# immars/parameter_server

Hardware: AMD Instinct MI355X
Metric: examples/sec (whole node) sparse LR 10^9 feats at 1/2/4/8 MI355X (higher is better)
Workload: dtype fp32; 1 GPU; global_batch=65536, seq_len=39, nnz_per_example=39, parallelism=dp1+kvshard1, consistency=bsp (1 shard: every pull sees every earlier push), table_slots_per_gpu=2147483648, hip_graph=False, collectives_in_graphs=False, prep_streams=3, localize=tpf

## Files before the change

### parameter_server_amd/csrc/hip/tploc.cuh

```cuda
#pragma once
#include "tploc.h"

namespace psamd {

namespace tp {
constexpr int kThr = 1024;
constexpr int kIt = 8;
constexpr int kTile = kThr * kIt;
constexpr int kHash = 2 * kTile;
constexpr int kHB = 14;
constexpr int kDispB = 12;
constexpr uint32_t kMaxDisp = (1u << kDispB) - 1;
constexpr int kMaxBk = 2048;
constexpr int kMaxT = 640;
constexpr int kBThr = 256;
constexpr int kBkThr = 512;
constexpr int kECap = 4096;
constexpr int kECapL = 4064;
constexpr int kDH = 2048;
constexpr int kBkProbe = 128;
constexpr uint32_t kEmpty = 0xffffffffu;
constexpr int kG = (kECapL + kBkThr - 1) / kBkThr;
}

__device__ __forceinline__ uint32_t tp_hash(uint32_t x) {
  x ^= x >> 16;
  x *= 0x7feb352du;
  x ^= x >> 15;
  x *= 0x846ca68bu;
  x ^= x >> 16;
  return x;
}

template <int kN>
__device__ __forceinline__ uint32_t tp_block_scan(uint32_t v, uint32_t* lds, uint32_t* total) {
  constexpr int kW = kN / 64;
  const int lane = threadIdx.x & 63, wid = threadIdx.x >> 6;
  uint32_t x = v;
#pragma unroll
  for (int off = 1; off < 64; off <<= 1) {
    const uint32_t y = __shfl_up(x, off, 64);
    if (lane >= off) x += y;
  }
  if (lane == 63) lds[wid] = x;
  __syncthreads();
  if (threadIdx.x == 0) {
    uint32_t run = 0;
    for (int w = 0; w < kW; ++w) {
      const uint32_t t = lds[w];
      lds[w] = run;
      run += t;
    }
    lds[kW] = run;
  }
  __syncthreads();
  const uint32_t r = x - v + lds[wid];
  *total = lds[kW];
  __syncthreads();
  return r;
}

template <int kN>
__device__ __forceinline__ uint32_t tp_prefix(const uint32_t* __restrict__ a, int b, uint32_t* lds) {
  uint32_t s = 0;
  for (int i = threadIdx.x; i < b; i += kN) s += a[i];
  uint32_t tot;
  tp_block_scan<kN>(s, lds, &tot);
  return tot;
}

__device__ __forceinline__ uint64_t tp_match_any(uint32_t v, int nbits, uint64_t active) {
  uint64_t peers = active;
  for (int b = 0; b < nbits; ++b) {
    const bool bit = (v >> b) & 1u;
    const uint64_t bal = __ballot(bit);
    peers &= bit ? bal : ~bal;
  }
  return peers;
}

template <bool kCnt = false>
__device__ __forceinline__ bool tp_bk_build(const uint32_t* __restrict__ tkeys,
                                            const uint16_t* __restrict__ toff, int nbf, int T,
                                            int shift, int f0, int nf, uint32_t hb,
                                            uint32_t* hkey, uint32_t* hcnt, uint64_t* dl,
                                            uint16_t* eh, uint32_t* lds, uint32_t* flag,
                                            int32_t (&idx)[tp::kG], uint32_t* E_out,
                                            uint32_t* D_out, uint64_t* prof,
                                            const uint8_t* __restrict__ ecnt = nullptr) {
  using namespace tp;
  const int t = threadIdx.x;
  uint32_t* tpre = reinterpret_cast<uint32_t*>(dl);
  uint16_t* tlo = reinterpret_cast<uint16_t*>(tpre + kMaxT + 1);
  uint16_t* tmid = tlo + kMaxT;
  for (int s = t; s < kDH; s += kBkThr) {
    hkey[s] = kEmpty;
    hcnt[s] = 0;
  }
  if (t == 0) *flag = 0;
  const int per = (T + kBkThr - 1) / kBkThr;
  const int q0 = t * per, q1 = q0 + per < T ? q0 + per : T;
  uint32_t c = 0;
  for (int q = q0; q < q1; ++q) {
    const uint16_t* to = toff + (int64_t)q * (nbf + 1);
    const uint32_t lo = to[f0], hi = to[f0 + nf];
    tlo[q] = (uint16_t)lo;
    tmid[q] = (uint16_t)((nf == 2 ? to[f0 + 1] : hi) - lo);
    tpre[q] = hi - lo;
    c += hi - lo;
  }
  uint32_t E;
  uint32_t w = tp_block_scan<kBkThr>(c, lds, &E);
  for (int q = q0; q < q1; ++q) {
    const uint32_t len = tpre[q];
    tpre[q] = w;
    w += len;
  }
  if (t == 0) tpre[T] = E;
  __syncthreads();
  if (prof && t == 0) prof[(int64_t)blockIdx.x * 12 + 1] = clock64();
  const uint32_t En = E < (uint32_t)kECapL ? E : (uint32_t)kECapL;
  bool bad = E > (uint32_t)kECapL;
  uint32_t hib = 0;
#pragma unroll
  for (int q = 0; q < kG; ++q) {
    const uint32_t g = q * kBkThr + t;
    idx[q] = -1;
    if (g < En) {
      int lo = 0, up = T - 1;
      while (lo < up) {
        const int mid = (lo + up + 1) >> 1;
        if (tpre[mid] <= g) lo = mid; else up = mid - 1;
      }
      const uint32_t off = g - tpre[lo];
      idx[q] = lo * kTile + tlo[lo] + (int32_t)off;
      hib |= (off >= tmid[lo] ? 1u : 0u) << q;
    }
  }
  uint32_t kv[kG];
  uint32_t ecp[(kG + 3) / 4];
#pragma unroll
  for (int q = 0; q < kG; ++q) kv[q] = idx[q] >= 0 ? tkeys[idx[q]] : 0u;
  if (kCnt) {
#pragma unroll
    for (int w = 0; w < (kG + 3) / 4; ++w) ecp[w] = 0u;
#pragma unroll
    for (int q = 0; q < kG; ++q)
      if (idx[q] >= 0) ecp[q >> 2] |= (uint32_t)ecnt[idx[q]] << ((q & 3) * 8);
  }
#pragma unroll
  for (int q = 0; q < kG; ++q) {
    if (idx[q] < 0) continue;
    const uint32_t g = q * kBkThr + t;
    const uint32_t key = kv[q] | ((hb + ((hib >> q) & 1u)) << shift);
    uint32_t h = tp_hash(key) & (kDH - 1);
    bool ok = false;
    bad |= __hip_atomic_load(flag, __ATOMIC_RELAXED, __HIP_MEMORY_SCOPE_WORKGROUP) != 0u;
    for (int p = 0; p < kBkProbe && !bad; ++p) {
      const uint32_t cu = hkey[h];
      if (cu == kEmpty) {
        const uint32_t prev = atomicCAS(&hkey[h], kEmpty, key);
        if (prev == kEmpty || prev == key) { ok = true; break; }
      } else if (cu == key) {
        ok = true;
        break;
      }
      h = (h + 1) & (kDH - 1);
    }
    if (ok) {
      atomicAdd(&hcnt[h], kCnt ? (ecp[q >> 2] >> ((q & 3) * 8)) & 0xffu : 1u);
    } else if (!bad) {
      bad = true;
      atomicOr(flag, 1u);
    }
    eh[g] = ok ? (uint16_t)h : (uint16_t)0xffffu;
  }
  if (bad) atomicOr(flag, 1u);
  __syncthreads();
  if (prof && t == 0) prof[(int64_t)blockIdx.x * 12 + 2] = clock64();
  constexpr int kPer = kDH / kBkThr;
  uint64_t ent[kPer];
  uint32_t cc = 0;
#pragma unroll
  for (int q = 0; q < kPer; ++q) {
    const int s = q * kBkThr + t;
    ent[q] = hkey[s] != kEmpty
                 ? (((uint64_t)hkey[s] << 32) |
                    ((uint64_t)(kCnt ? min(hcnt[s], 0xffffu) : hcnt[s]) << 16) | (uint64_t)s)
                 : ~0ull;
    cc += ent[q] != ~0ull;
  }
  uint32_t D;
  uint32_t wd = tp_block_scan<kBkThr>(cc, lds, &D);
#pragma unroll
  for (int q = 0; q < kPer; ++q)
    if (ent[q] != ~0ull) dl[wd++] = ent[q];
  *E_out = En;
  *D_out = D;
  const bool good = *flag == 0u;
  __syncthreads();
  return good;
}

__device__ __forceinline__ void tp_bk_ranksort(uint64_t* dl, uint64_t* hs, uint32_t D) {
  using namespace tp;
  const int t = threadIdx.x;
  if (t < 8 && D + t < (uint32_t)kDH) dl[D + t] = ~0ull;
  uint32_t* rk = reinterpret_cast<uint32_t*>(hs + 1024);
  const int tpk = D <= 128 ? 4 : D <= 256 ? 2 : 1;
  if (tpk > 1 && t < 256) rk[t] = 0;
  __syncthreads();
  const uint4* d4 = reinterpret_cast<const uint4*>(dl);
  const uint32_t nq = (D + 7) / 8;
  if (tpk > 1) {
    const int nk = kBkThr / tpk, i = t % nk, h = t / nk;
    const uint32_t pq = (nq + tpk - 1) / tpk;
    const uint32_t qa = h * pq, qb = qa + pq < nq ? qa + pq : nq;
    if ((uint32_t)i < D) {
      const uint64_t x = dl[i];
      uint32_t r = 0;
      for (uint32_t q = qa; q < qb; ++q) {
        uint4 v[4];
#pragma unroll
        for (int k = 0; k < 4; ++k) v[k] = d4[q * 4 + k];
#pragma unroll
        for (int k = 0; k < 4; ++k) {
          r += (((uint64_t)v[k].y << 32) | v[k].x) < x;
          r += (((uint64_t)v[k].w << 32) | v[k].z) < x;
        }
      }
      atomicAdd(&rk[i], r);
    }
    __syncthreads();
    if (h == 0 && (uint32_t)i < D) hs[rk[i]] = dl[i];
  } else {
    for (uint32_t i = t; i < D; i += kBkThr) {
      const uint64_t x = dl[i];
      uint32_t r = 0;
      for (uint32_t q = 0; q < nq; ++q) {
        uint4 v[4];
#pragma unroll
        for (int k = 0; k < 4; ++k) v[k] = d4[q * 4 + k];
#pragma unroll
        for (int k = 0; k < 4; ++k) {
          r += (((uint64_t)v[k].y << 32) | v[k].x) < x;
          r += (((uint64_t)v[k].w << 32) | v[k].z) < x;
        }
      }
      hs[r] = x;
    }
  }
}

__device__ __forceinline__ int fx_shift(uint32_t maxbits) {
  int e = 0;
  if (maxbits) (void)frexpf(__uint_as_float(maxbits), &e);
  return min(100, 48 - e);
}
__device__ __forceinline__ void fx_add(long long* acc, int idx, float v, double sc) {
  const long long fx = __double2ll_rn((double)v * sc);
  if (fx) atomicAdd(reinterpret_cast<unsigned long long*>(&acc[idx]), (unsigned long long)fx);
}
__device__ __forceinline__ void fx_tile_max(float vmax, uint32_t* smax) {
  vmax = wave_max(vmax);
  if ((threadIdx.x & 63) == 0 && vmax > 0.f) atomicMax(smax, __float_as_uint(vmax));
}

namespace tpf {
constexpr int kUnitK = tp::kDH;
constexpr int kUC = 2 * kUnitK;
constexpr int kEC = 8192;
constexpr int kThr = 256;
constexpr uint32_t kNoSlot = 0xffffffffu;
}

__host__ __device__ __forceinline__ int tpf_xcd_group_of(int bid, int groups) {
  if (groups < 8) return bid;
  const int q = groups >> 3, r = groups & 7, xcd = bid & 7;
  const int base = xcd < r ? xcd * (q + 1) : r * (q + 1) + (xcd - r) * q;
  return base + (bid >> 3);
}

}
```

### parameter_server_amd/csrc/hip/tploc.hip

```cpp
#include "tploc.cuh"
#include "tploc_geom.h"

#include <algorithm>
#include <cstdlib>

namespace psamd {

__device__ uint64_t* g_tile_prof = nullptr;
#define TILE_MARK(k)                                                            \
  if (tpp && threadIdx.x == 0) tpp[(int64_t)blockIdx.x * 16 + (k)] = clock64()

template <bool kQuot, bool kCnt = false>
__global__ void __launch_bounds__(tp::kThr, 8)
tp_tile_kernel(const uint64_t* __restrict__ raw, int64_t n, KeyMix m, int shift, int nbk,
               uint32_t* __restrict__ tkeys, uint16_t* __restrict__ toff,
               int32_t* __restrict__ dcnt, uint16_t* __restrict__ rep,
               int32_t* __restrict__ err, int lts, uint8_t* __restrict__ ecnt = nullptr) {
  using namespace tp;
  __shared__ uint32_t hk[kHash];
  __shared__ uint32_t cnt[kMaxBk];
  __shared__ uint32_t lds[kThr / 64 + 1];
  const int t = threadIdx.x;
  uint64_t* const tpp = g_tile_prof;
  if (tpp && t == 0) tpp[(int64_t)blockIdx.x * 16 + 8] = __builtin_amdgcn_s_memrealtime();
  TILE_MARK(0);
  for (int i = t; i < kHash; i += kThr) hk[i] = kEmpty;
  for (int d = t; d < nbk; d += kThr) cnt[d] = 0;
  __syncthreads();
  TILE_MARK(1);
  const int64_t base = (int64_t)blockIdx.x << lts;
  const int lim = (int)(n - base < (1 << lts) ? n - base : (1 << lts));
  uint64_t kr[kIt];
  uint16_t sl[kIt];
  uint32_t rr[kIt];
  uint32_t won = 0;
  bool bad = false;
#pragma unroll
  for (int j = 0; j < kIt; ++j) {
    const int o = j * kThr + t;
    kr[j] = o < lim ? raw[base + o] : 0ull;
  }
  if (tpp) {
    __builtin_amdgcn_s_waitcnt(0);
    __syncthreads();
    TILE_MARK(2);
  }
#pragma unroll
  for (int j = 0; j < kIt; ++j) {
    sl[j] = 0;
    if (j * kThr + t < lim) {
      const uint64_t k = kQuot ? mix_key(kr[j], m) : (uint64_t)mix_key32(kr[j], m);
      kr[j] = k;
      const uint32_t q = kQuot ? (uint32_t)(k >> kHB) << kDispB : (uint32_t)k;
      uint32_t h = (uint32_t)k & (kHash - 1);
      uint32_t d = 0;
      for (; d < kMaxDisp; ++d) {
        const uint32_t want = kQuot ? q | d : q;
        const uint32_t cur = hk[h];
        if (cur == want) break;
        if (cur == kEmpty) {
          const uint32_t prev = atomicCAS(&hk[h], kEmpty, want);
          if (prev == kEmpty) {
            won |= 1u << j;
            break;
          }
          if (prev == want) break;
        }
        h = (h + 1) & (kHash - 1);
      }
      bad |= d == kMaxDisp;
      sl[j] = (uint16_t)h;
    }
  }
#pragma unroll
  for (int j = 0; j < kIt; ++j)
    rr[j] = (won >> j) & 1u ? atomicAdd(&cnt[kr[j] >> shift], 1u) : kEmpty;
  if (bad && err) atomicOr(err, 2);
  __syncthreads();
  TILE_MARK(3);
  constexpr int kDP = kMaxBk / kThr;
  uint32_t c[kDP], s = 0;
#pragma unroll
  for (int e = 0; e < kDP; ++e) {
    const int d = t * kDP + e;
    c[e] = d < nbk ? cnt[d] : 0u;
    s += c[e];
  }
  uint32_t D;
  uint32_t run = tp_block_scan<kThr>(s, lds, &D);
  uint16_t* to = toff + (int64_t)blockIdx.x * (nbk + 1);
#pragma unroll
  for (int e = 0; e < kDP; ++e) {
    const int d = t * kDP + e;
    if (d < nbk) {
      cnt[d] = run;
      to[d] = (uint16_t)run;
    }
    run += c[e];
  }
  if (t == 0) {
    to[nbk] = (uint16_t)D;
    dcnt[blockIdx.x] = (int32_t)D;
  }
  __syncthreads();
  TILE_MARK(4);
  uint32_t* tk = tkeys + (int64_t)blockIdx.x * kTile;
  const uint64_t smask = (1ull << shift) - 1;
#pragma unroll
  for (int j = 0; j < kIt; ++j) {
    if (rr[j] != kEmpty) {
      const uint32_t pos = cnt[kr[j] >> shift] + rr[j];
      tk[pos] = (uint32_t)(kr[j] & smask);
      hk[sl[j]] = pos;
    }
  }
  __syncthreads();
  TILE_MARK(5);
#pragma unroll
  for (int j = 0; j < kIt; ++j) {
    const int o = j * kThr + t;
    if (o < lim) {
      const uint16_t pos = (uint16_t)hk[sl[j]];
      rep[base + o] = pos;
      if (kCnt) sl[j] = pos;
    }
  }
  if (kCnt) {
    __syncthreads();
    for (uint32_t i = t; i < (D + 1) / 2; i += kThr) hk[i] = 0u;
    __syncthreads();
#pragma unroll
    for (int j = 0; j < kIt; ++j)
      if (j * kThr + t < lim) atomicAdd(&hk[sl[j] >> 1], 1u << ((sl[j] & 1) * 16));
    __syncthreads();
    uint8_t* ec = ecnt + (int64_t)blockIdx.x * kTile;
    for (uint32_t i = t; i < D; i += kThr) {
      const uint32_t c = (hk[i >> 1] >> ((i & 1) * 16)) & 0xffffu;
      ec[i] = (uint8_t)(c > 255u ? 255u : c);
    }
  }
  if (tpp && t == 0) {
    TILE_MARK(6);
    tpp[(int64_t)blockIdx.x * 16 + 9] = __builtin_amdgcn_s_memrealtime();
    tpp[(int64_t)blockIdx.x * 16 + 10] = __smid();
  }
}
#undef TILE_MARK

void tp_tile_set_prof(uint64_t* p) {
  PSAMD_HIP_CHECK(hipMemcpyToSymbol(HIP_SYMBOL(g_tile_prof), &p, sizeof(p)));
}

__global__ void tp_gather_kernel(const uint16_t* __restrict__ rep,
                                 const int32_t* __restrict__ ent_uid, int64_t n,
                                 int32_t* __restrict__ local_col) {
  constexpr int kPer = 4;
  const int64_t i0 = (blockIdx.x * (int64_t)blockDim.x) * kPer + threadIdx.x;
  int64_t e[kPer];
#pragma unroll
  for (int q = 0; q < kPer; ++q) {
    const int64_t i = i0 + q * blockDim.x;
    e[q] = i < n ? (i / tp::kTile) * tp::kTile + rep[i] : -1;
  }
#pragma unroll
  for (int q = 0; q < kPer; ++q) {
    const int64_t i = i0 + q * blockDim.x;
    if (e[q] >= 0) local_col[i] = ent_uid[e[q]];
  }
}

int tp_flat_lts(int64_t n) {
  const char* pe = getenv("PSAMD_TILE_LTS");
  const int pin = pe ? atoi(pe) : 0;
  const char* te = getenv("PSAMD_TILE_MIN");
  int tmin = te ? atoi(te) : 128;
  tmin = tmin < 1 ? 1 : tmin > tp::kMaxT / 2 ? tp::kMaxT / 2 : tmin;
  int lts = 13;
  if (pin >= 10 && pin <= 13) {
    lts = pin;
  } else {
    while (lts > 10 && ((n + (1ll << lts) - 1) >> lts) < tmin) --lts;
  }
  while (lts < 13 && ((n + (1ll << lts) - 1) >> lts) > tp::kMaxT) ++lts;
  return lts;
}

TpGeom tp_geom(int64_t n, int bits, bool flat) {
  TpGeom g;
  g.lts = flat ? tp_flat_lts(n) : 13;
  static_assert(tp::kTile == 8192, "tile entry stride 2^13");
  g.T = (n + (1ll << g.lts) - 1) >> g.lts;
  g.N = g.T * tp::kTile;
  int bb = 0;
  while (bb < 11 && (n >> bb) > 1024) ++bb;
  if (bb > bits) bb = bits;
  g.nbk = 1 << bb;
  g.shift = bits - bb;
  return g;
}

int64_t tploc_stride(int64_t n) { return tp_geom(n, 31).N; }
int64_t tpf_stride(int64_t n) { return tp_geom(n, 31, true).N; }
int64_t tpf_stride_max(int64_t n) {
  const int64_t t = std::min<int64_t>(tp::kMaxT, (n + 1023) / 1024);
  return std::max<int64_t>(t, (n + tp::kTile - 1) / tp::kTile) * tp::kTile;
}
int tpf_tile_log2(int64_t n) { return tp_geom(n, 31, true).lts; }
int tploc_buckets(int64_t n, int bits) { return tp_geom(n, bits).nbk; }
int tploc_tile() { return tp::kTile; }

bool tploc_supported(int64_t n, int bits) {
  return bits >= 2 && bits <= 34 && n > 0 && (n >> 11) <= 1280 &&
         (n + tp::kTile - 1) / tp::kTile <= tp::kMaxT && tp_geom(n, bits).shift <= 31;
}

size_t tploc_temp_bytes(int64_t n, int bits) {
  const TpGeom g = tp_geom(n, bits);
  return al16((size_t)g.nbk * 8 + 16)
         + al16((size_t)g.N * 4)
         + al16((size_t)g.T * (g.nbk + 1) * 2);
}

void tp_launch_tile(const uint64_t* raw, int64_t n, KeyMix m, const TpGeom& g, uint32_t* tkeys,
                    uint16_t* toff, int32_t* dcnt, uint16_t* rep, int32_t* err, uint8_t* ecnt,
                    hipStream_t st) {
  auto launch = [&](auto kernel) {
    kernel<<<(unsigned)g.T, tp::kThr, 0, st>>>(raw, n, m, g.shift, g.nbk, tkeys, toff, dcnt, rep,
                                               err, g.lts, ecnt);
  };
  const bool quot = m.bits > 31;
  if (quot && ecnt) launch(tp_tile_kernel<true, true>);
  else if (ecnt) launch(tp_tile_kernel<false, true>);
  else if (quot) launch(tp_tile_kernel<true, false>);
  else launch(tp_tile_kernel<false, false>);
  PSAMD_HIP_CHECK(hipGetLastError());
}

int tpf_groups(int64_t n, int bits) { return tpf_groups_of(tp_geom(n, bits)); }
int tpf_key_region() { return tpf::kUC; }
int tpf_entry_region() { return tpf::kEC; }
int tpf_xcd_group(int bid, int groups) { return tpf_xcd_group_of(bid, groups); }

size_t tpf_temp_bytes(int64_t n, int bits) {
  const int64_t N = tpf_stride_max(n);
  return al16((size_t)N * 4) + al16((size_t)(N / tp::kTile) * (tp::kMaxBk + 1) * 2);
}

void tp_gather(const uint16_t* rep, const int32_t* ent_uid, int64_t n, int32_t* local_col,
               hipStream_t st) {
  if (n <= 0) return;
  tp_gather_kernel<<<(unsigned)((n + 1023) / 1024), 256, 0, st>>>(rep, ent_uid, n, local_col);
  PSAMD_HIP_CHECK(hipGetLastError());
}

}
```

### parameter_server_amd/csrc/hip/tploc_bucket.hip

```cpp
#include "tploc.cuh"
#include "tploc_geom.h"

#include <stdexcept>

namespace psamd {

namespace tp {
constexpr uint64_t kStA = 1, kStP = 2;
constexpr uint32_t kStM = (1u << 27) - 1;
}
__device__ __forceinline__ uint64_t tp_status(uint32_t ep, uint64_t flag, uint32_t d, uint32_t e) {
  return ((uint64_t)ep << 56) | (flag << 54) | ((uint64_t)(d & tp::kStM) << 27) | (e & tp::kStM);
}

__device__ __forceinline__ void tp_bk_emit(const uint64_t* hs, uint64_t* dl, const uint16_t* eh,
                                           const int32_t (&idx)[tp::kG], uint32_t D,
                                           uint32_t ubase, uint32_t ebase, uint64_t key0,
                                           uint32_t* lds, int32_t* __restrict__ pos_s,
                                           int32_t* __restrict__ segid,
                                           uint64_t* __restrict__ uniq,
                                           int32_t* __restrict__ seg_start,
                                           int32_t* __restrict__ ent_uid,
                                           float* __restrict__ zero_a,
                                           unsigned long long* __restrict__ zero_b,
                                           int64_t u_cap, int64_t e_cap, uint64_t* prof) {
  using namespace tp;
  const int t = threadIdx.x;
  uint32_t* cur = reinterpret_cast<uint32_t*>(dl);
  uint16_t* jj = reinterpret_cast<uint16_t*>(cur + kDH);
  __syncthreads();
  uint32_t carry = 0;
  for (uint32_t j0 = 0; j0 < D; j0 += kBkThr) {
    const uint32_t j = j0 + t;
    const uint64_t v = j < D ? hs[j] : 0ull;
    const uint32_t cnt = (uint32_t)(v >> 16) & 0xffffu;
    uint32_t tot;
    const uint32_t ex = tp_block_scan<kBkThr>(cnt, lds, &tot) + carry;
    if (j < D) {
      const uint32_t slot = (uint32_t)v & 0xffffu;
      const int64_t u = (int64_t)ubase + j;
      if (in_range(u, u_cap)) {
        uniq[u] = key0 | (uint32_t)(v >> 32);
        seg_start[u] = (int32_t)(ebase + ex);
        if (zero_a) zero_a[u] = 0.f;
        if (zero_b) zero_b[u] = 0ull;
      }
      cur[slot] = ex;
      jj[slot] = (uint16_t)j;
    }
    carry += tot;
  }
  __syncthreads();
  if (prof && t == 0) prof[(int64_t)blockIdx.x * 12 + 6] = clock64();
#pragma unroll
  for (int q = 0; q < kG; ++q) {
    if (idx[q] < 0) continue;
    const uint32_t h = eh[q * kBkThr + t];
    if (h == 0xffffu) continue;
    const uint32_t pos = atomicAdd(&cur[h], 1u);
    const uint32_t u = ubase + jj[h];
    const int64_t e = (int64_t)ebase + pos;
    if (in_range(e, e_cap)) {
      pos_s[e] = idx[q];
      segid[e] = (int32_t)(u + 1);
    }
    if (in_range((int64_t)idx[q], e_cap)) ent_uid[idx[q]] = (int32_t)u;
  }
  __syncthreads();
}

__device__ __forceinline__ void tp_bk_lookback(uint64_t* __restrict__ status, int fs, int twin,
                                               int nbf, uint32_t ep, uint32_t D, uint32_t E,
                                               uint32_t* sb, uint32_t* __restrict__ epoch,
                                               int32_t* __restrict__ n_uniq,
                                               int32_t* __restrict__ n_ent,
                                               int32_t* __restrict__ seg_start, int64_t u_cap,
                                               int32_t* __restrict__ err) {
  using namespace tp;
  const int lane = threadIdx.x;
  if (lane >= 64) return;
  uint32_t su = 0, se = 0;
  if (fs > 0) {
    int j = fs - 1;
    uint32_t spins = 0;
    while (true) {
      const int jl = j - lane;
      const uint64_t st =
          jl >= 0 ? __hip_atomic_load(&status[jl], __ATOMIC_RELAXED, __HIP_MEMORY_SCOPE_AGENT)
                  : tp_status(ep, kStP, 0, 0);
      const uint32_t f = (uint32_t)(st >> 56) == ep ? (uint32_t)(st >> 54) & 3u : 0u;
      const uint64_t pm = __ballot(f == kStP), nr = __ballot(f == 0);
      const int fp = pm ? __builtin_ctzll(pm) : 64;
      const uint64_t need = fp >= 63 ? ~0ull : ((2ull << fp) - 1);
      if (nr & need) {
        if (++spins > (1u << 22)) {
          if (lane == 0) atomicOr(err, 4);
          break;
        }
        __builtin_amdgcn_s_sleep(1);
        continue;
      }
      const bool inc = lane <= fp;
      su += wave_allsum(inc ? (uint32_t)(st >> 27) & kStM : 0u);
      se += wave_allsum(inc ? (uint32_t)st & kStM : 0u);
      if (fp < 64) break;
      j -= 64;
    }
  }
  if (lane == 0) {
    const uint64_t inc = tp_status(ep, kStP, su + D, se + E);
    if (fs > 0) __hip_atomic_store(&status[fs], inc, __ATOMIC_RELAXED, __HIP_MEMORY_SCOPE_AGENT);
    if (twin != fs) __hip_atomic_store(&status[twin], inc, __ATOMIC_RELAXED, __HIP_MEMORY_SCOPE_AGENT);
    sb[1] = su;
    sb[2] = se;
    if (twin == nbf - 1) {
      const uint32_t U = su + D, Et = se + E;
      *n_uniq = (int32_t)U;
      *n_ent = (int32_t)Et;
      if (in_range((int64_t)U, u_cap + 1)) seg_start[U] = (int32_t)Et;
      __hip_atomic_store(epoch, ep, __ATOMIC_RELAXED, __HIP_MEMORY_SCOPE_AGENT);
    }
  }
}

__device__ __forceinline__ void tp_bk_fine_light(
    const uint32_t* __restrict__ tkeys, const uint16_t* __restrict__ toff, int nbf, int T,
    int shift, int f, uint32_t hb, uint64_t key0, uint32_t* hkey, uint32_t* hcnt, uint64_t* hs,
    uint64_t* dl, uint16_t* ehraw, uint32_t* lds, uint32_t* sb, uint64_t* __restrict__ status,
    uint32_t ep, uint32_t* __restrict__ epoch, int32_t* __restrict__ pos_s,
    int32_t* __restrict__ segid, uint64_t* __restrict__ uniq, int32_t* __restrict__ seg_start,
    int32_t* __restrict__ ent_uid, int32_t* __restrict__ n_uniq, int32_t* __restrict__ n_ent,
    float* __restrict__ zero_a, unsigned long long* __restrict__ zero_b, int64_t u_cap,
    int64_t e_cap, int32_t* __restrict__ err) {
  using namespace tp;
  static_assert((kMaxT + 1) * 4 + kMaxT * 2 <= kECapL * 2, "tile runs must fit in eh");
  const int t = threadIdx.x;
  uint32_t* tpre = reinterpret_cast<uint32_t*>(ehraw);
  uint16_t* tlo = reinterpret_cast<uint16_t*>(tpre + kMaxT + 1);
  for (int s = t; s < kDH; s += kBkThr) {
    hkey[s] = kEmpty;
    hcnt[s] = 0;
  }
  const int per = (T + kBkThr - 1) / kBkThr;
  const int q0 = t * per, q1 = q0 + per < T ? q0 + per : T;
  uint32_t c = 0;
  for (int q = q0; q < q1; ++q) {
    const uint16_t* to = toff + (int64_t)q * (nbf + 1);
    const uint32_t lo = to[f], hi = to[f + 1];
    tlo[q] = (uint16_t)lo;
    tpre[q] = hi - lo;
    c += hi - lo;
  }
  uint32_t E;
  uint32_t w = tp_block_scan<kBkThr>(c, lds, &E);
  for (int q = q0; q < q1; ++q) {
    const uint32_t len = tpre[q];
    tpre[q] = w;
    w += len;
  }
  if (t == 0) tpre[T] = E;
  __syncthreads();
  auto locate = [&](uint32_t g) -> int32_t {
    int lo = 0, up = T - 1;
    while (lo < up) {
      const int mid = (lo + up + 1) >> 1;
      if (tpre[mid] <= g) lo = mid; else up = mid - 1;
    }
    return lo * kTile + tlo[lo] + (int32_t)(g - tpre[lo]);
  };
  bool bad = false;
  for (uint32_t g = t; g < E; g += kBkThr) {
    const uint32_t key = tkeys[locate(g)] | (hb << shift);
    uint32_t h = tp_hash(key) & (kDH - 1);
    bool ok = false;
    for (int p = 0; p < kBkProbe && !bad; ++p) {
      const uint32_t cu = hkey[h];
      if (cu == kEmpty) {
        const uint32_t prev = atomicCAS(&hkey[h], kEmpty, key);
        if (prev == kEmpty || prev == key) { ok = true; break; }
      } else if (cu == key) {
        ok = true;
        break;
      }
      h = (h + 1) & (kDH - 1);
    }
    if (ok) atomicAdd(&hcnt[h], 1u);
    else bad = true;
  }
  if (bad) atomicOr(err, 1);
  __syncthreads();
  constexpr int kPer = kDH / kBkThr;
  uint32_t cc = 0;
  for (int q = 0; q < kPer; ++q) cc += hkey[q * kBkThr + t] != kEmpty;
  uint32_t D;
  uint32_t wd = tp_block_scan<kBkThr>(cc, lds, &D);
  for (int q = 0; q < kPer; ++q) {
    const int s = q * kBkThr + t;
    if (hkey[s] != kEmpty) dl[wd++] = ((uint64_t)hkey[s] << 32) | ((uint64_t)hcnt[s] << 16) | (uint64_t)s;
  }
  if (t == 0)
    __hip_atomic_store(&status[f], tp_status(ep, f == 0 ? kStP : kStA, D, E), __ATOMIC_RELAXED,
                       __HIP_MEMORY_SCOPE_AGENT);
  __syncthreads();
  tp_bk_ranksort(dl, hs, D);
  tp_bk_lookback(status, f, f, nbf, ep, D, E, sb, epoch, n_uniq, n_ent, seg_start, u_cap, err);
  __syncthreads();
  const uint32_t ubase = sb[1], ebase = sb[2];
  uint32_t* cur = reinterpret_cast<uint32_t*>(dl);
  uint32_t carry = 0;
  for (uint32_t j0 = 0; j0 < D; j0 += kBkThr) {
    const uint32_t j = j0 + t;
    const uint64_t v = j < D ? hs[j] : 0ull;
    const uint32_t cnt = (uint32_t)(v >> 16) & 0xffffu;
    uint32_t tot;
    const uint32_t ex = tp_block_scan<kBkThr>(cnt, lds, &tot) + carry;
    if (j < D) {
      const int64_t u = (int64_t)ubase + j;
      if (in_range(u, u_cap)) {
        uniq[u] = key0 | (uint32_t)(v >> 32);
        seg_start[u] = (int32_t)(ebase + ex);
        if (zero_a) zero_a[u] = 0.f;
        if (zero_b) zero_b[u] = 0ull;
      }
      cur[j] = ex;
    }
    carry += tot;
  }
  __syncthreads();
  for (uint32_t g = t; g < E; g += kBkThr) {
    const int32_t id = locate(g);
    const uint32_t key = tkeys[id] | (hb << shift);
    uint32_t lo = 0, up = D - 1;
    while (lo < up) {
      const uint32_t mid = (lo + up) >> 1;
      if ((uint32_t)(hs[mid] >> 32) < key) lo = mid + 1; else up = mid;
    }
    if (D == 0 || (uint32_t)(hs[lo] >> 32) != key) continue;
    const uint32_t pos = atomicAdd(&cur[lo], 1u);
    const uint32_t u = ubase + lo;
    const int64_t e = (int64_t)ebase + pos;
    if (in_range(e, e_cap)) {
      pos_s[e] = id;
      segid[e] = (int32_t)(u + 1);
    }
    if (in_range((int64_t)id, e_cap)) ent_uid[id] = (int32_t)u;
  }
  __syncthreads();
}

__global__ void __launch_bounds__(tp::kBkThr, 8)
tp_bucket_kernel(const uint32_t* __restrict__ tkeys, const uint16_t* __restrict__ toff, int nbf,
                 int pair, int T, int shift, uint64_t* __restrict__ status,
                 uint32_t* __restrict__ epoch, int32_t* __restrict__ pos_s,
                 int32_t* __restrict__ segid, uint64_t* __restrict__ uniq,
                 int32_t* __restrict__ seg_start, int32_t* __restrict__ ent_uid,
                 int32_t* __restrict__ n_uniq, int32_t* __restrict__ n_ent,
                 float* __restrict__ zero_a, unsigned long long* __restrict__ zero_b,
                 int64_t u_cap, int64_t e_cap, int32_t* __restrict__ err,
                 uint64_t* __restrict__ prof) {
  using namespace tp;
  __shared__ uint16_t eh[kECapL];
  __shared__ uint64_t hs[kDH];
  __shared__ uint64_t dl[kDH];
  __shared__ uint32_t lds[kBkThr / 64 + 1];
  __shared__ uint32_t sb[4];
  static_assert((kMaxT + 1) * 4 + kMaxT * 4 <= kDH * 8, "tile runs must fit in dl");
  uint32_t* hkey = reinterpret_cast<uint32_t*>(hs);
  uint32_t* hcnt = hkey + kDH;
  const int t = threadIdx.x, b = blockIdx.x;
  if (prof && t == 0) {
    prof[(int64_t)b * 12 + 0] = clock64();
    prof[(int64_t)b * 12 + 8] = __builtin_amdgcn_s_memrealtime();
  }
  if (t == 0) {
    uint32_t ep = (__hip_atomic_load(epoch, __ATOMIC_RELAXED, __HIP_MEMORY_SCOPE_AGENT) + 1u) & 0xffu;
    sb[0] = ep ? ep : 1u;
  }
  const int f0 = pair ? 2 * b : b, twin = pair ? f0 + 1 : f0;
  const uint64_t key0 = (uint64_t)f0 << shift;
  int32_t idx[kG];
  uint32_t E, D;
  const bool good = tp_bk_build(tkeys, toff, nbf, T, shift, f0, pair ? 2 : 1, 0u, hkey, hcnt, dl,
                                eh, lds, &sb[3], idx, &E, &D, prof);
  const uint32_t ep = sb[0];
  if (!good && pair) {
#pragma unroll 1
    for (int s = 0; s < 2; ++s)
      tp_bk_fine_light(tkeys, toff, nbf, T, shift, f0 + s, (uint32_t)s, key0, hkey, hcnt, hs, dl,
                       eh, lds, sb, status, ep, epoch, pos_s, segid, uniq, seg_start, ent_uid,
                       n_uniq, n_ent, zero_a, zero_b, u_cap, e_cap, err);
    return;
  }
  if (!good && t == 0) atomicOr(err, 1);
  if (t == 0) {
    if (twin != f0)
      __hip_atomic_store(&status[twin], tp_status(ep, kStA, 0, 0), __ATOMIC_RELAXED,
                         __HIP_MEMORY_SCOPE_AGENT);
    __hip_atomic_store(&status[f0], tp_status(ep, f0 == 0 ? kStP : kStA, D, E), __ATOMIC_RELAXED,
                       __HIP_MEMORY_SCOPE_AGENT);
  }
  if (prof && t == 0) prof[(int64_t)b * 12 + 3] = clock64();
  tp_bk_ranksort(dl, hs, D);
  if (prof && t == 0) prof[(int64_t)b * 12 + 4] = clock64();
  tp_bk_lookback(status, f0, twin, nbf, ep, D, E, sb, epoch, n_uniq, n_ent, seg_start, u_cap, err);
  __syncthreads();
  if (prof && t == 0) prof[(int64_t)b * 12 + 5] = clock64();
  tp_bk_emit(hs, dl, eh, idx, D, sb[1], sb[2], key0, lds, pos_s, segid, uniq, seg_start, ent_uid,
             zero_a, zero_b, u_cap, e_cap, prof);
  if (prof && t == 0) {
    prof[(int64_t)b * 12 + 7] = clock64();
    prof[(int64_t)b * 12 + 9] = __builtin_amdgcn_s_memrealtime();
  }
}

__device__ __forceinline__ uint32_t tpf_unit_light(
    const uint32_t* __restrict__ tkeys, const uint16_t* __restrict__ toff, int nbf, int T,
    int shift, int f, uint32_t hb, uint64_t key0, uint32_t* hkey, uint32_t* hmap,
    uint16_t* ehraw, uint32_t* lds, uint64_t* __restrict__ uo, int32_t* __restrict__ po,
    uint16_t* __restrict__ jo, uint32_t eoff, int32_t* __restrict__ co,
    int32_t* __restrict__ err, bool sorted) {
  using namespace tp;
  const int t = threadIdx.x;
  uint32_t* tpre = reinterpret_cast<uint32_t*>(ehraw);
  uint16_t* tlo = reinterpret_cast<uint16_t*>(tpre + kMaxT + 1);
  for (int s = t; s < kDH; s += kBkThr) hkey[s] = kEmpty;
  const int per = (T + kBkThr - 1) / kBkThr;
  const int q0 = t * per, q1 = q0 + per < T ? q0 + per : T;
  uint32_t c = 0;
  for (int q = q0; q < q1; ++q) {
    const uint16_t* to = toff + (int64_t)q * (nbf + 1);
    const uint32_t lo = to[f], hi = to[f + 1];
    tlo[q] = (uint16_t)lo;
    tpre[q] = hi - lo;
    c += hi - lo;
  }
  uint32_t E;
  uint32_t w = tp_block_scan<kBkThr>(c, lds, &E);
  for (int q = q0; q < q1; ++q) {
    const uint32_t len = tpre[q];
    tpre[q] = w;
    w += len;
  }
  if (t == 0) tpre[T] = E;
  __syncthreads();
  auto locate = [&](uint32_t g) -> int32_t {
    int lo = 0, up = T - 1;
    while (lo < up) {
      const int mid = (lo + up + 1) >> 1;
      if (tpre[mid] <= g) lo = mid; else up = mid - 1;
    }
    return lo * kTile + tlo[lo] + (int32_t)(g - tpre[lo]);
  };
  auto probe = [&](uint32_t key, bool insert) -> int {
    uint32_t h = tp_hash(key) & (kDH - 1);
    for (int p = 0; p < kDH; ++p) {
      const uint32_t cu = hkey[h];
      if (cu == key) return (int)h;
      if (cu == kEmpty) {
        if (!insert) return -1;
        const uint32_t prev = atomicCAS(&hkey[h], kEmpty, key);
        if (prev == kEmpty || prev == key) return (int)h;
      }
      h = (h + 1) & (kDH - 1);
    }
    return -1;
  };
  bool bad = false;
  constexpr int kLB = 4;
  for (uint32_t c0 = 0; c0 < E; c0 += kBkThr * kLB) {
    int32_t id[kLB];
    uint32_t kk[kLB];
#pragma unroll
    for (int q = 0; q < kLB; ++q) {
      const uint32_t g = c0 + q * kBkThr + t;
      id[q] = locate(g < E ? g : E - 1);
    }
#pragma unroll
    for (int q = 0; q < kLB; ++q) kk[q] = tkeys[id[q]];
#pragma unroll
    for (int q = 0; q < kLB; ++q)
      if (c0 + q * kBkThr + t < E) bad |= probe(kk[q] | (hb << shift), true) < 0;
  }
  __syncthreads();
  constexpr int kPer = kDH / kBkThr;
  uint32_t cc = 0;
#pragma unroll
  for (int q = 0; q < kPer; ++q) cc += hkey[q * kBkThr + t] != kEmpty;
  uint32_t D;
  uint32_t wd = tp_block_scan<kBkThr>(cc, lds, &D);
#pragma unroll
  for (int q = 0; q < kPer; ++q) {
    const int s = q * kBkThr + t;
    const uint32_t k = hkey[s];
    if (k != kEmpty) {
      uint32_t j = wd++;
      if (sorted) {
        j = 0;
        for (int r = 0; r < kDH; ++r) j += hkey[r] < k;
      }
      hmap[s] = j;
      uo[j] = key0 | k;
    }
  }
  __syncthreads();
  const uint32_t room = eoff < (uint32_t)tpf::kEC ? tpf::kEC - eoff : 0u;
  bad |= E > room;
  const uint32_t Er = E < room ? E : room;
  for (uint32_t c0 = 0; c0 < Er; c0 += kBkThr * kLB) {
    int32_t id[kLB];
    uint32_t kk[kLB];
#pragma unroll
    for (int q = 0; q < kLB; ++q) {
      const uint32_t g = c0 + q * kBkThr + t;
      id[q] = locate(g < Er ? g : Er - 1);
    }
#pragma unroll
    for (int q = 0; q < kLB; ++q) kk[q] = tkeys[id[q]];
#pragma unroll
    for (int q = 0; q < kLB; ++q) {
      const uint32_t g = c0 + q * kBkThr + t;
      if (g >= Er) continue;
      const int h = probe(kk[q] | (hb << shift), false);
      po[eoff + g] = id[q];
      jo[eoff + g] = h >= 0 ? (uint16_t)hmap[h] : (uint16_t)0;
    }
  }
  if (bad) atomicOr(err, 1);
  if (t == 0) {
    co[0] = (int32_t)D;
    co[1] = (int32_t)(E < room ? E : room);
  }
  __syncthreads();
  return E < room ? E : room;
}

__device__ __forceinline__ void tpf_rank_binned(uint64_t* dl, uint32_t* sc, uint32_t D, int kbits,
                                                uint32_t* lds) {
  using namespace tp;
  constexpr int kPerT = kDH / kBkThr;
  const int t = threadIdx.x;
  const int bsh = kbits > 8 ? kbits - 8 : 0;
  uint32_t* bkey = sc;
  uint32_t* bcnt = sc + kDH;
  uint32_t* bst = bcnt + 256;
  if (t < 256) bcnt[t] = 0u;
  __syncthreads();
  uint64_t e[kPerT];
  uint32_t bs[kPerT];
#pragma unroll
  for (int q = 0; q < kPerT; ++q) {
    const uint32_t i = q * kBkThr + t;
    e[q] = i < D ? dl[i] : 0ull;
    if (i < D) {
      const uint32_t bin = ((uint32_t)(e[q] >> 32) >> bsh) & 255u;
      bs[q] = bin << 16 | atomicAdd(&bcnt[bin], 1u);
    }
  }
  __syncthreads();
  uint32_t tot;
  const uint32_t st = tp_block_scan<kBkThr>(t < 256 ? bcnt[t] : 0u, lds, &tot);
  if (t < 256) bst[t] = st;
  __syncthreads();
#pragma unroll
  for (int q = 0; q < kPerT; ++q)
    if (q * kBkThr + t < D) bkey[bst[bs[q] >> 16] + (bs[q] & 0xffffu)] = (uint32_t)(e[q] >> 32);
  __syncthreads();
  uint32_t rk[kPerT];
#pragma unroll
  for (int q = 0; q < kPerT; ++q) {
    if (q * kBkThr + t >= D) continue;
    const uint32_t bin = bs[q] >> 16, a = bst[bin], n = bcnt[bin];
    const uint32_t k = (uint32_t)(e[q] >> 32);
    uint32_t r = a;
    for (uint32_t m = 0; m < n; ++m) r += bkey[a + m] < k;
    rk[q] = r;
  }
  __syncthreads();
#pragma unroll
  for (int q = 0; q < kPerT; ++q)
    if (q * kBkThr + t < D) dl[rk[q]] = e[q];
  __syncthreads();
}

template <bool kFilt>
__global__ void __launch_bounds__(tp::kBkThr, 8)
tpf_bucket_kernel(const uint32_t* __restrict__ tkeys, const uint16_t* __restrict__ toff, int nbf,
                  int pair, int T, int shift, uint64_t* __restrict__ uniqf,
                  int32_t* __restrict__ ent_pos, uint16_t* __restrict__ ent_j,
                  int32_t* __restrict__ cnt, int32_t* __restrict__ err, int sorted,
                  const uint8_t* __restrict__ ecnt) {
  using namespace tp;
  __shared__ alignas(16) uint16_t eh[kECapL];
  __shared__ uint64_t hs[kDH];
  __shared__ uint64_t dl[kDH];
  __shared__ uint32_t lds[kBkThr / 64 + 1];
  __shared__ uint32_t flag;
  uint32_t* hkey = reinterpret_cast<uint32_t*>(hs);
  uint32_t* hcnt = hkey + kDH;
  const int t = threadIdx.x, b = blockIdx.x;
  const int f0 = pair ? 2 * b : b;
  const uint64_t key0 = (uint64_t)f0 << shift;
  uint64_t* uo = uniqf + (int64_t)b * tpf::kUC;
  int32_t* po = ent_pos + (int64_t)b * tpf::kEC;
  uint16_t* jo = ent_j + (int64_t)b * tpf::kEC;
  int32_t* co = cnt + (int64_t)b * 4;
  int32_t idx[kG];
  uint32_t E, D;
  const bool good = tp_bk_build<kFilt>(tkeys, toff, nbf, T, shift, f0, pair ? 2 : 1, 0u, hkey,
                                       hcnt, dl, eh, lds, &flag, idx, &E, &D, nullptr, ecnt);
  if (good) {
    uint32_t* jmap = hcnt;
    const uint64_t* lst = dl;
    if (sorted && D > 64) {
      tpf_rank_binned(dl, hkey, D, pair ? shift + 1 : shift, lds);
      jmap = hkey;
    } else if (sorted) {
      tp_bk_ranksort(dl, hs, D);
      __syncthreads();
      jmap = reinterpret_cast<uint32_t*>(dl);
      lst = hs;
    }
    for (uint32_t j = t; j < D; j += kBkThr) {
      const uint64_t v = lst[j];
      uo[j] = key0 | (uint32_t)(v >> 32) |
              (kFilt ? (uint64_t)min((uint32_t)(v >> 16) & 0xffffu, 255u) << 56 : 0ull);
      jmap[(uint32_t)v & 0xffffu] = j;
    }
    __syncthreads();
#pragma unroll
    for (int q = 0; q < kG; ++q) {
      if (idx[q] < 0) continue;
      const uint32_t g = q * kBkThr + t;
      po[g] = idx[q];
      jo[g] = (uint16_t)jmap[eh[g]];
    }
    if (t == 0) {
      co[0] = (int32_t)D;
      co[1] = (int32_t)E;
      co[2] = 0;
      co[3] = 0;
    }
  } else {
    {
      const uint32_t e0 = tpf_unit_light(tkeys, toff, nbf, T, shift, f0, 0u, key0, hkey, hcnt, eh,
                                         lds, uo, po, jo, 0u, co, err, sorted != 0);
      if (pair)
        tpf_unit_light(tkeys, toff, nbf, T, shift, f0 + 1, 1u, key0, hkey, hcnt, eh, lds,
                       uo + tpf::kUnitK, po, jo, e0, co + 2, err, sorted != 0);
      else if (t == 0) {
        co[2] = 0;
        co[3] = 0;
      }
    }
  }
}

void localize_tp(const uint64_t* raw, int64_t n, KeyMix m, void* temp, size_t temp_bytes,
                 int32_t* dcnt, uint16_t* rep, int32_t* pos_s, int32_t* segid, uint64_t* uniq,
                 int32_t* seg_start, int32_t* ent_uid, int32_t* local_col, int32_t* n_uniq,
                 int32_t* n_ent, float* grad, unsigned long long* pieces, int32_t* err,
                 int64_t u_cap, uint64_t* prof, hipStream_t st) {
  if (n <= 0) return;
  if (!tploc_supported(n, m.bits)) throw std::runtime_error("localize_tp: unsupported size");
  if (temp_bytes < tploc_temp_bytes(n, m.bits)) throw std::runtime_error("localize_tp: temp");
  const TpGeom g = tp_geom(n, m.bits);
  char* p = (char*)temp;
  auto take = [&](size_t bytes) { char* r = p; p += al16(bytes); return r; };
  uint64_t* status = (uint64_t*)take((size_t)g.nbk * 8 + 16);
  uint32_t* epoch = (uint32_t*)(status + g.nbk);
  uint32_t* tkeys = (uint32_t*)take((size_t)g.N * 4);
  uint16_t* toff = (uint16_t*)take((size_t)g.T * (g.nbk + 1) * 2);
  tp_launch_tile(raw, n, m, g, tkeys, toff, dcnt, rep, err, nullptr, st);
  const bool pair = g.nbk >= 2 && g.shift <= 30;
  tp_bucket_kernel<<<(unsigned)(pair ? g.nbk / 2 : g.nbk), tp::kBkThr, 0, st>>>(
      tkeys, toff, g.nbk, pair ? 1 : 0, (int)g.T, g.shift, status, epoch, pos_s, segid, uniq,
      seg_start, ent_uid, n_uniq, n_ent, grad, pieces, u_cap, g.N, err, prof);
  PSAMD_HIP_CHECK(hipGetLastError());
  if (local_col) tp_gather(rep, ent_uid, n, local_col, st);
}

void tpf_launch_bucket(const TpGeom& g, const uint32_t* tkeys, const uint16_t* toff,
                       uint64_t* uniqf, int32_t* ent_pos, uint16_t* ent_j, int32_t* cnt,
                       int32_t* err, bool sorted, const uint8_t* ecnt, hipStream_t st) {
  const int pair = tpf_pair(g) ? 1 : 0;
  if (ecnt)
    tpf_bucket_kernel<true><<<(unsigned)tpf_groups_of(g), tp::kBkThr, 0, st>>>(
        tkeys, toff, g.nbk, pair, (int)g.T, g.shift, uniqf, ent_pos, ent_j, cnt, err,
        sorted ? 1 : 0, ecnt);
  else
    tpf_bucket_kernel<false><<<(unsigned)tpf_groups_of(g), tp::kBkThr, 0, st>>>(
        tkeys, toff, g.nbk, pair, (int)g.T, g.shift, uniqf, ent_pos, ent_j, cnt, err,
        sorted ? 1 : 0, nullptr);
  PSAMD_HIP_CHECK(hipGetLastError());
}

}
```

Before: 903.1 million examples/sec.

## Restructure tile hash insert and skip unused bucket counts

The tile localize kernel now issues the raw key loads before clearing the shared hash table, so load latency overlaps the init. Key and slot state is packed into 32-bit registers, and each key gets one speculative CAS at its home slot before a linear probe that runs only for collided keys. The bucket build gains a mode that skips the hcnt zeroing and atomic count increments when counts are not needed (the non-filter path). Register pressure and the probe loop's serial dependence should drop, at the cost of more complex bit-packing and a changed probe structure that could alter behaviour at the displacement limit.

```diff
diff --git a/parameter_server_amd/csrc/hip/tploc.cuh b/parameter_server_amd/csrc/hip/tploc.cuh
--- a/parameter_server_amd/csrc/hip/tploc.cuh
+++ b/parameter_server_amd/csrc/hip/tploc.cuh
@@ -79,7 +79,8 @@
   return peers;
 }
 
-template <bool kCnt = false>
+enum class BkCount { kNone, kEntries, kOcc };
+template <BkCount kMode = BkCount::kEntries>
 __device__ __forceinline__ bool tp_bk_build(const uint32_t* __restrict__ tkeys,
                                             const uint16_t* __restrict__ toff, int nbf, int T,
                                             int shift, int f0, int nf, uint32_t hb,
@@ -89,13 +90,14 @@
                                             uint32_t* D_out, uint64_t* prof,
                                             const uint8_t* __restrict__ ecnt = nullptr) {
   using namespace tp;
+  constexpr bool kCnt = kMode == BkCount::kOcc;
   const int t = threadIdx.x;
   uint32_t* tpre = reinterpret_cast<uint32_t*>(dl);
   uint16_t* tlo = reinterpret_cast<uint16_t*>(tpre + kMaxT + 1);
   uint16_t* tmid = tlo + kMaxT;
   for (int s = t; s < kDH; s += kBkThr) {
     hkey[s] = kEmpty;
-    hcnt[s] = 0;
+    if (kMode != BkCount::kNone) hcnt[s] = 0;
   }
   if (t == 0) *flag = 0;
   const int per = (T + kBkThr - 1) / kBkThr;
@@ -168,7 +170,8 @@
       h = (h + 1) & (kDH - 1);
     }
     if (ok) {
-      atomicAdd(&hcnt[h], kCnt ? (ecp[q >> 2] >> ((q & 3) * 8)) & 0xffu : 1u);
+      if (kMode != BkCount::kNone)
+        atomicAdd(&hcnt[h], kCnt ? (ecp[q >> 2] >> ((q & 3) * 8)) & 0xffu : 1u);
     } else if (!bad) {
       bad = true;
       atomicOr(flag, 1u);
@@ -186,7 +189,10 @@
     const int s = q * kBkThr + t;
     ent[q] = hkey[s] != kEmpty
                  ? (((uint64_t)hkey[s] << 32) |
-                    ((uint64_t)(kCnt ? min(hcnt[s], 0xffffu) : hcnt[s]) << 16) | (uint64_t)s)
+                    (kMode == BkCount::kNone
+                         ? 0ull
+                         : (uint64_t)(kCnt ? min(hcnt[s], 0xffffu) : hcnt[s]) << 16) |
+                    (uint64_t)s)
                  : ~0ull;
     cc += ent[q] != ~0ull;
   }
diff --git a/parameter_server_amd/csrc/hip/tploc.hip b/parameter_server_amd/csrc/hip/tploc.hip
--- a/parameter_server_amd/csrc/hip/tploc.hip
+++ b/parameter_server_amd/csrc/hip/tploc.hip
@@ -24,14 +24,19 @@
   uint64_t* const tpp = g_tile_prof;
   if (tpp && t == 0) tpp[(int64_t)blockIdx.x * 16 + 8] = __builtin_amdgcn_s_memrealtime();
   TILE_MARK(0);
-  for (int i = t; i < kHash; i += kThr) hk[i] = kEmpty;
-  for (int d = t; d < nbk; d += kThr) cnt[d] = 0;
-  __syncthreads();
-  TILE_MARK(1);
   const int64_t base = (int64_t)blockIdx.x << lts;
-  const int lim = (int)(n - base < (1 << lts) ? n - base : (1 << lts));
+  const int lim = __builtin_amdgcn_readfirstlane(
+      (int)(n - base < (1 << lts) ? n - base : (1 << lts)));
   uint64_t kr[kIt];
-  uint16_t sl[kIt];
+  uint32_t kl[kIt], kh = 0;
+  auto key = [&](int j) {
+    return kQuot ? (uint64_t)((kh >> (4 * j)) & 0xfu) << 32 | kl[j] : (uint64_t)kl[j];
+  };
+  uint32_t sl2[kIt / 2] = {};
+  auto sl = [&](int j) { return (sl2[j >> 1] >> ((j & 1) * 16)) & 0xffffu; };
+  auto set_sl = [&](int j, uint32_t v) {
+    sl2[j >> 1] = (sl2[j >> 1] & (0xffff0000u >> ((j & 1) * 16))) | v << ((j & 1) * 16);
+  };
   uint32_t rr[kIt];
   uint32_t won = 0;
   bool bad = false;
@@ -40,41 +45,65 @@
     const int o = j * kThr + t;
     kr[j] = o < lim ? raw[base + o] : 0ull;
   }
+  for (int i = t; i < kHash; i += kThr) hk[i] = kEmpty;
+  for (int d = t; d < nbk; d += kThr) cnt[d] = 0;
+  __syncthreads();
+  TILE_MARK(1);
   if (tpp) {
     __builtin_amdgcn_s_waitcnt(0);
     __syncthreads();
     TILE_MARK(2);
   }
-#pragma unroll
-  for (int j = 0; j < kIt; ++j) {
-    sl[j] = 0;
-    if (j * kThr + t < lim) {
+  uint32_t vm = 0;
+  uint32_t pv[kIt];
+#pragma unroll
+  for (int j = 0; j < kIt; ++j) {
+    pv[j] = 0u;
+    kl[j] = 0u;
+    if (j * kThr < lim) {
+      const bool valid = j * kThr + t < lim;
+      vm |= (valid ? 1u : 0u) << j;
       const uint64_t k = kQuot ? mix_key(kr[j], m) : (uint64_t)mix_key32(kr[j], m);
-      kr[j] = k;
+      kl[j] = (uint32_t)k;
+      if (kQuot) kh |= (uint32_t)(k >> 32) << (4 * j);
+      const uint32_t h = valid ? (uint32_t)k & (kHash - 1) : (uint32_t)t;
+      set_sl(j, h);
       const uint32_t q = kQuot ? (uint32_t)(k >> kHB) << kDispB : (uint32_t)k;
-      uint32_t h = (uint32_t)k & (kHash - 1);
-      uint32_t d = 0;
-      for (; d < kMaxDisp; ++d) {
-        const uint32_t want = kQuot ? q | d : q;
-        const uint32_t cur = hk[h];
-        if (cur == want) break;
+      pv[j] = atomicCAS(&hk[h], kEmpty, valid ? q : kEmpty);
+    }
+  }
+  uint32_t coll = 0;
+#pragma unroll
+  for (int j = 0; j < kIt; ++j) {
+    const uint32_t q = kQuot ? (uint32_t)(key(j) >> kHB) << kDispB : kl[j];
+    won |= (pv[j] == kEmpty ? 1u : 0u) << j;
+    coll |= (pv[j] != kEmpty && pv[j] != q ? 1u : 0u) << j;
+  }
+  won &= vm;
+  coll &= vm;
+#pragma unroll
+  for (int j = 0; j < kIt; ++j) {
+    if ((coll >> j) & 1u) {
+      const uint32_t q = kQuot ? (uint32_t)(key(j) >> kHB) << kDispB : kl[j];
+      uint32_t h = sl(j), d = 0, cur, want;
+      do {
+        ++d;
+        h = (h + 1) & (kHash - 1);
+        want = kQuot ? q | d : q;
+        cur = hk[h];
         if (cur == kEmpty) {
-          const uint32_t prev = atomicCAS(&hk[h], kEmpty, want);
-          if (prev == kEmpty) {
-            won |= 1u << j;
-            break;
-          }
-          if (prev == want) break;
+          cur = atomicCAS(&hk[h], kEmpty, want);
+          won |= (cur == kEmpty ? 1u : 0u) << j;
+          cur = cur == kEmpty ? want : cur;
         }
-        h = (h + 1) & (kHash - 1);
-      }
-      bad |= d == kMaxDisp;
-      sl[j] = (uint16_t)h;
+      } while (cur != want && d < kMaxDisp - 1);
+      bad |= cur != want;
+      set_sl(j, h);
     }
   }
 #pragma unroll
   for (int j = 0; j < kIt; ++j)
-    rr[j] = (won >> j) & 1u ? atomicAdd(&cnt[kr[j] >> shift], 1u) : kEmpty;
+    rr[j] = (won >> j) & 1u ? atomicAdd(&cnt[key(j) >> shift], 1u) : kEmpty;
   if (bad && err) atomicOr(err, 2);
   __syncthreads();
   TILE_MARK(3);
@@ -109,9 +138,9 @@
 #pragma unroll
   for (int j = 0; j < kIt; ++j) {
     if (rr[j] != kEmpty) {
-      const uint32_t pos = cnt[kr[j] >> shift] + rr[j];
-      tk[pos] = (uint32_t)(kr[j] & smask);
-      hk[sl[j]] = pos;
+      const uint32_t pos = cnt[key(j) >> shift] + rr[j];
+      tk[pos] = kl[j] & (uint32_t)smask;
+      hk[sl(j)] = pos;
     }
   }
   __syncthreads();
@@ -120,9 +149,9 @@
   for (int j = 0; j < kIt; ++j) {
     const int o = j * kThr + t;
     if (o < lim) {
-      const uint16_t pos = (uint16_t)hk[sl[j]];
+      const uint16_t pos = (uint16_t)hk[sl(j)];
       rep[base + o] = pos;
-      if (kCnt) sl[j] = pos;
+      if (kCnt) set_sl(j, pos);
     }
   }
   if (kCnt) {
@@ -131,7 +160,7 @@
     __syncthreads();
 #pragma unroll
     for (int j = 0; j < kIt; ++j)
-      if (j * kThr + t < lim) atomicAdd(&hk[sl[j] >> 1], 1u << ((sl[j] & 1) * 16));
+      if (j * kThr + t < lim) atomicAdd(&hk[sl(j) >> 1], 1u << ((sl(j) & 1) * 16));
     __syncthreads();
     uint8_t* ec = ecnt + (int64_t)blockIdx.x * kTile;
     for (uint32_t i = t; i < D; i += kThr) {
diff --git a/parameter_server_amd/csrc/hip/tploc_bucket.hip b/parameter_server_amd/csrc/hip/tploc_bucket.hip
--- a/parameter_server_amd/csrc/hip/tploc_bucket.hip
+++ b/parameter_server_amd/csrc/hip/tploc_bucket.hip
@@ -506,8 +506,9 @@
   int32_t* co = cnt + (int64_t)b * 4;
   int32_t idx[kG];
   uint32_t E, D;
-  const bool good = tp_bk_build<kFilt>(tkeys, toff, nbf, T, shift, f0, pair ? 2 : 1, 0u, hkey,
-                                       hcnt, dl, eh, lds, &flag, idx, &E, &D, nullptr, ecnt);
+  const bool good = tp_bk_build<kFilt ? BkCount::kOcc : BkCount::kNone>(
+      tkeys, toff, nbf, T, shift, f0, pair ? 2 : 1, 0u, hkey, hcnt, dl, eh, lds, &flag, idx, &E, &D,
+      nullptr, ecnt);
   if (good) {
     uint32_t* jmap = hcnt;
     const uint64_t* lst = dl;
@@ -527,10 +528,12 @@
       jmap[(uint32_t)v & 0xffffu] = j;
     }
     __syncthreads();
+    int to = t;
+    asm volatile("" : "+v"(to));
 #pragma unroll
     for (int q = 0; q < kG; ++q) {
       if (idx[q] < 0) continue;
-      const uint32_t g = q * kBkThr + t;
+      const uint32_t g = q * kBkThr + to;
       po[g] = idx[q];
       jo[g] = (uint16_t)jmap[eh[g]];
     }
```

Measured after the change: 862.0 million examples/sec. 0.955x the previous value.
